# AnnaLew/pangenomix

Hardware: AMD Instinct MI355X
Metric: proteins/sec clustered at 0.8 identity + pan/core iters/sec, 400-genome set (higher is better)
Workload: dtype i32

## Files before the change

### pangenomix_amd/csrc/cluster.hip

```cpp
#include <algorithm>
#include <chrono>
#include <cstdlib>
#include <cmath>
#include <type_traits>
#include <functional>
#include <condition_variable>
#include <mutex>
#include <thread>
#include <vector>

#include "cluster_layout.h"
#include "cluster_tables.h"
#include "pgx_internal.h"

namespace {

using namespace pgxc;

constexpr uint32_t kWindowMax = 65536;
constexpr int kDiscoveryRounds = 2;
constexpr uint32_t kBlockCap = 4096;
constexpr uint32_t kBlockCapMin = 64;

constexpr uint32_t kMaxLen = 1u << 22;
// ... 1583 lines not shown
        }
        if (lane == 0) {
            uint32_t fl = F_EVAL;
            if (best_sum >= req_aas[k1r]) fl |= F_DIAG_PASS;
            if (!(br >= len2 || bl <= -len1 || bl > br)) fl |= F_BAND_OK;
            if (br - bl + 1 > kMaxBand) { fl |= F_TOO_BIG; if (fl & F_DIAG_PASS) atomicOr(err, (uint32_t)E_BAND); }
            pairs[p].best_sum = best_sum; pairs[p].band_left = bl; pairs[p].band_center = bc;
            pairs[p].band_right = br; pairs[p].flags = fl;
        }
        __syncthreads();
    }
}

enum { BK_NONE = 0, BK_DIAG = 1, BK_LEFT = 2, BK_TOP = 3 };

__device__ __forceinline__ int64_t shfl_i64(int64_t v, int src_lane) {
    const int lo = __shfl((int)(uint32_t)v, src_lane);
    const int hi = __shfl((int)(v >> 32), src_lane);
    return (int64_t)(((uint64_t)(uint32_t)hi << 32) | (uint32_t)lo);
}

__device__ int band_align_wave(const uint8_t *__restrict__ s1, const uint8_t *__restrict__ s2, int len1,
                               int len2, int bl, int bc, int br, const int8_t *__restrict__ sub ,
                               int gap_open, int gap_ext) {
    const int lane = threadIdx.x & 63;
    const int bw = br - bl + 1;
    const int j1 = lane;
    const bool col = j1 < bw;
    const int i_start = max(1, 1 - bl - j1);
    const int i_end = min(len1, len2 - bl - j1);
    const int i_start_left = max(1, 2 - bl - j1);
    const int maxd = bc - bl;
    const int dist = j1 > maxd ? j1 - maxd : maxd - j1;
    const int64_t bonus = 4 - (dist & 3);
    const int64_t gap = kScoreScale * gap_open, ext = kScoreScale * gap_ext;
    int64_t sc = 0;
    int bk = BK_NONE, id = 0;
    const int t_last = 2 * len1 + bw - 1;
    for (int t = 2; t <= t_last; ++t) {
        const int64_t l_sc_n = shfl_i64(sc, (lane + 63) & 63);
        const int l_meta = __shfl((id << 2) | bk, (lane + 63) & 63);
        const int64_t r_sc_n = shfl_i64(sc, (lane + 1) & 63);
        const int r_meta = __shfl((id << 2) | bk, (lane + 1) & 63);
        const int d = t - j1;
        const int i = d >> 1;
        if (col && !(d & 1) && i >= i_start && i <= i_end) {
            const int j = j1 + i + bl;
            const int ci = s1[i - 1], cj = s2[j - 1];
            int64_t sij = kScoreScale * (int64_t)sub[ci * kNAA1 + cj];
            if (sij > 0) sij += bonus;
            int64_t p_sc; int p_id;
            if (i - 1 >= i_start) { p_sc = sc; p_id = id; }
            else { p_sc = ext * (int64_t)((i - 1 == 0) ? (j - 1) : (i - 1)); p_id = 0; }
            int64_t best = p_sc + sij;
            int back = BK_DIAG, nid = p_id + (ci == cj);
            const int64_t gap0 = (i == len1 || j == len2) ? ext : gap;
            if (j1 > 0) {
                int64_t l_sc; int l_bk, l_id;
                if (i >= i_start_left) { l_sc = l_sc_n; l_bk = l_meta & 3; l_id = l_meta >> 2; }
                else { l_sc = ext * (int64_t)i; l_bk = BK_NONE; l_id = 0; }
                const int64_t s = l_sc + (l_bk == BK_LEFT ? ext : gap0);
                if (s > best) { best = s; back = BK_LEFT; nid = l_id; }
            }
            if (j1 + 1 < bw) {
                int64_t r_sc; int r_bk, r_id;
                if (i - 1 >= 1) { r_sc = r_sc_n; r_bk = r_meta & 3; r_id = r_meta >> 2; }
                else { r_sc = ext * (int64_t)j; r_bk = BK_NONE; r_id = 0; }
                const int64_t s = r_sc + (r_bk == BK_TOP ? ext : gap0);
                if (s > best) { best = s; back = BK_TOP; nid = r_id; }
            }
            sc = best; bk = back; id = nid;
        }
    }
    int end_lane;
    if (len2 - bl < len1) end_lane = 0;
    else if (len1 + br < len2) end_lane = bw - 1;
    else end_lane = len2 - len1 - bl;
    return __shfl(id, end_lane);
}

constexpr int kA16MaxSlot = 4096;
constexpr int kA16BigSlot = 8192;
constexpr int kScaleShift = 14;

__device__ __forceinline__ int dpp_row_shr1(int v) { return __builtin_amdgcn_update_dpp(0, v, 0x111, 0xF, 0xF, true); }
__device__ __forceinline__ int dpp_row_shl1(int v) { return __builtin_amdgcn_update_dpp(0, v, 0x101, 0xF, 0xF, true); }

__device__ __forceinline__ uint32_t lane_select(uint64_t mask, uint32_t if_set, uint32_t if_clear) {
    uint32_t d;
    asm("v_cndmask_b32_e64 %0, %1, %2, %3" : "=v"(d) : "v"(if_clear), "v"(if_set), "s"(mask));
    return d;
}
__device__ __forceinline__ uint64_t lanes_equal(uint32_t a, uint32_t b) { return __builtin_amdgcn_uicmp(a, b, 32 ); }

__device__ __forceinline__ bool pair_is_wide(int len1, int len2, int bl, int br, int max_sum) {
    return len1 + len2 > max_sum || br - bl + 1 > 32;
}

template <int kA16Slot>
__global__ __launch_bounds__(256) void align16_kernel(DevSeqs S, const uint32_t *__restrict__ rep_seq,
                                                     Pair *__restrict__ pairs, PairSel sel,
                                                     const int32_t *__restrict__ req_aa1, double cluster_thd,
                                                     uint32_t b0, unsigned long long *__restrict__ best,
                                                     uint32_t key_flag, uint32_t *__restrict__ n_wide, uint32_t second_pass) {
    __shared__ int2 tab[4][kNAA1 * kNAA1];
    __shared__ uint32_t seqbuf[16 * (kA16Slot / 4) + 32];
    __builtin_amdgcn_s_setprio(3);
    const uint32_t n = sel_count(sel);
    if (blockIdx.x * 16u >= n) return;
    if (second_pass && *n_wide == 0u) return;
    for (int c = threadIdx.x; c < 4 * kNAA1 * kNAA1; c += 256) {
        const int cc = c % (kNAA1 * kNAA1);
        const int s = S.nt ? (cc / kNAA1 == cc % kNAA1 ? 2 : -2) : (int)kBlosum62_dev[cc];
        const int v = s * (1 << kScaleShift) + (s > 0 ? c / (kNAA1 * kNAA1) + 1 : 0);
        tab[c / (kNAA1 * kNAA1)][cc] = make_int2(v * 4 + 2, cc / kNAA1 == cc % kNAA1);
    }
    __syncthreads();
    const int lane = threadIdx.x & 63, gl = lane & 15;
    const int slot = (threadIdx.x >> 6) * 4 + (lane >> 4);
    const uint8_t *sb = reinterpret_cast<const uint8_t *>(seqbuf + slot * (kA16Slot / 4));
    const int gap = (S.nt ? -6 : kGapOpen) * (1 << kScaleShift), ext = (S.nt ? -1 : kGapExt) * (1 << kScaleShift);
    constexpr int kNever = INT32_MIN / 2;

    for (uint32_t base = blockIdx.x * 16u; base < n; base += gridDim.x * 16u) {
        const uint32_t w = base + (uint32_t)slot;
        uint32_t p = 0;
        Pair pr{};
        bool fast = false;
        int len1 = 1, len2 = 1;
        uint32_t k1 = 0, k2 = 0;
        if (w < n) {
            p = sel_pair(sel, w);
            pr = pairs[p];
            k1 = pr.q; k2 = rep_seq ? rep_seq[pr.r] : pr.r;
            len1 = (int)S.len[k1]; len2 = (int)S.len[k2];
            fast = (pr.flags & (F_DIAG_PASS | F_BAND_OK | F_TOO_BIG | F_ALIGNED)) == (F_DIAG_PASS | F_BAND_OK);
            if (fast && pair_is_wide(len1, len2, pr.band_left, pr.band_right, kA16Slot - 96)) {
                fast = false;
                if (gl == 0 && !second_pass) atomicAdd(n_wide, 1u);
            }
        }
        const int bl = pr.band_left, bw = fast ? pr.band_right - pr.band_left + 1 : 0;
        int o1 = 0, o2 = 0;
        if (fast) {
            const uint32_t *p1 = S.pk + S.pk_off[k1], *p2 = S.pk + S.pk_off[k2];
            const int w1 = (len1 + 5) / 6, w2 = (len2 + 5) / 6;
            uint8_t *sbw = reinterpret_cast<uint8_t *>(seqbuf + slot * (kA16Slot / 4));
            o2 = (6 * w1 + 7) & ~7;
            for (int w = gl; w < w1; w += 16) {
                const uint32_t x = p1[w];
                for (int t = 0; t < 6; ++t) sbw[6 * w + t] = (uint8_t)((x >> (5 * t)) & 31u);
            }
            for (int w = gl; w < w2; w += 16) {
                const uint32_t x = p2[w];
                for (int t = 0; t < 6; ++t) sbw[o2 + 6 * w + t] = (uint8_t)(((x >> (5 * t)) & 31u) << 3);
            }
        }
        const int c0 = 2 * gl, c1 = c0 + 1;
        const bool v0 = c0 < bw, v1 = c1 < bw;
        const int if0 = max(0, -bl - c0), if1 = max(0, -bl - c1);
        const int ie0 = min(len1, len2 - bl - c0), ie1 = min(len1, len2 - bl - c1);
        const int bs0 = ext * (if0 > 0 ? if0 : c0 + bl), bs1 = ext * (if1 > 0 ? if1 : c1 + bl);
        const int maxd = pr.band_center - bl;
        const int d0 = c0 > maxd ? c0 - maxd : maxd - c0, d1 = c1 > maxd ? c1 - maxd : maxd - c1;
        const int2 *t0 = tab[3 - (d0 & 3)], *t1 = tab[3 - (d1 & 3)];
        const bool left0 = c0 > 0, top0 = c0 + 1 < bw, top1 = c1 + 1 < bw;
        const int trip = fast ? len1 + ((bw + 1) >> 1) : 0;

        auto res1 = [&](int i) { return (int)sb[o1 + max(i - 1, 0)]; };
        auto res2 = [&](int j) { return (int)sb[o2 + min(max(j - 1, 0), len2 - 1)]; };
        auto entry = [](const int2 *t, int c_query, int c_rep8) {
            return *reinterpret_cast<const int2 *>(__builtin_assume_aligned(
                reinterpret_cast<const char *>(t) + c_query * (kNAA1 * 8) + c_rep8, 8));
        };
        int i = -gl;
        int ci = res1(i), cje = res2(c0 + i + bl), cjo = res2(c1 + i + bl);
        int2 te = entry(t0, ci, cje), to = entry(t1, ci, cjo);
        int sc0 = 0, m0 = 0, sc1 = 0, m1 = 0;

        auto row = [&](int tau) {
            const int ci_n = res1(i + 1), cjo_n = res2(c1 + i + 1 + bl);
            const int cje_n = cjo;
            const int se = te.x >> 2, so = to.x >> 2, me = te.y, mo = to.y;
            const int l_sc = dpp_row_shr1(sc1), l_m = dpp_row_shr1(m1);
            {
                const int g0 = i == ie0 ? ext : gap;
                int bst = sc0 + se, bm = ((m0 >> 2) + me) << 2 | BK_DIAG;
                const int ls = left0 ? l_sc + ((l_m & 3) == BK_LEFT ? ext : g0) : kNever;
                if (ls > bst) { bst = ls; bm = (l_m & ~3) | BK_LEFT; }
                const int ts = top0 ? sc1 + ((m1 & 3) == BK_TOP ? ext : g0) : kNever;
                if (ts > bst) { bst = ts; bm = (m1 & ~3) | BK_TOP; }
                if (i == if0) { bst = bs0; bm = BK_NONE; }
                if (v0 && tau < trip && i >= if0 && i <= ie0) { sc0 = bst; m0 = bm; }
            }
            const int r_sc = dpp_row_shl1(sc0), r_m = dpp_row_shl1(m0);
            {
                const int g0 = i == ie1 ? ext : gap;
                int bst = sc1 + so, bm = ((m1 >> 2) + mo) << 2 | BK_DIAG;
                const int ls = sc0 + ((m0 & 3) == BK_LEFT ? ext : g0);
                if (ls > bst) { bst = ls; bm = (m0 & ~3) | BK_LEFT; }
                const int ts = top1 ? r_sc + ((r_m & 3) == BK_TOP ? ext : g0) : kNever;
                if (ts > bst) { bst = ts; bm = (r_m & ~3) | BK_TOP; }
                if (i == if1) { bst = bs1; bm = BK_NONE; }
                if (v1 && tau < trip && i >= if1 && i <= ie1) { sc1 = bst; m1 = bm; }
            }
            __builtin_amdgcn_sched_barrier(0);
            cje = cje_n; cjo = cjo_n; ci = ci_n;
            te = entry(t0, ci, cje); to = entry(t1, ci, cjo);
            ++i;
        };
        int lo = 0, hi = INT32_MAX, wtrip = trip;
        if (fast && v0) {
            lo = max(if0, v1 ? if1 : 0) + gl + 1;
            hi = min(ie0, v1 ? ie1 : ie0) + gl;
        }
        for (int d = 32; d > 0; d >>= 1) {
            lo = max(lo, __shfl_xor(lo, d)); hi = min(hi, __shfl_xor(hi, d)); wtrip = max(wtrip, __shfl_xor(wtrip, d));
        }
        wtrip = __builtin_amdgcn_readfirstlane(wtrip);
        lo = __builtin_amdgcn_readfirstlane(min(lo, wtrip)); hi = __builtin_amdgcn_readfirstlane(min(hi, wtrip));
        int tau = 0;
        for (; tau < lo; ++tau) row(tau);
        if (tau < hi) {
            constexpr uint32_t kBias = 0x80000000u;
            uint32_t G1 = (uint32_t)(gap * 4 + 1), E1 = (uint32_t)(ext * 4 + 1), G0 = (uint32_t)(gap * 4), E0 = (uint32_t)(ext * 4);
            asm volatile("" : "+v"(G1), "+v"(E1), "+v"(G0), "+v"(E0));
            const uint32_t live0 = v0 ? ~0u : 0u, live1 = v1 ? ~0u : 0u;
            auto to_key = [&](int sc, int m, uint32_t live, uint32_t &K, uint32_t &N, uint32_t &XL, uint32_t &XT) {
                const uint32_t Kc = (uint32_t)(sc * 4) + kBias;
                const int b = m & 3;
                K = Kc | (b == BK_LEFT ? 1u : (b == BK_TOP ? 0u : 2u));
                N = (uint32_t)(m >> 2);
                XL = (Kc + (b == BK_LEFT ? E1 : G1)) & live;
                XT = (Kc + (b == BK_TOP ? E0 : G0)) & live;
            };
            uint32_t K0, N0, XL0, XT0, K1, N1, XL1, XT1;
            to_key(sc0, m0, live0, K0, N0, XL0, XT0);
            to_key(sc1, m1, live1, K1, N1, XL1, XT1);
            const uint8_t *a1 = sb + o1 + i, *a2 = sb + o2 + c1 + i + bl;
            auto step = [&]() {
                const int ci_n = *a1, cjo_n = *a2;
                const int cje_n = cjo;
                ++a1; ++a2;
                {
                    const uint32_t lXL = (uint32_t)__builtin_amdgcn_update_dpp(0, (int)XL1, 0x111, 0xF, 0xF, true);
                    const uint32_t lN = (uint32_t)dpp_row_shr1((int)N1);
                    const uint32_t K = max(max((K0 & ~3u) + (uint32_t)te.x, lXL), XT1);
                    const uint32_t b = K & 3u, Kc = K & ~3u;
                    const uint64_t isL = lanes_equal(b, 1u), isT = lanes_equal(b, 0u);
                    N0 = lane_select(isL, lN, lane_select(isT, N1, N0 + (uint32_t)te.y));
                    K0 = K;
                    XL0 = (Kc + lane_select(isL, E1, G1)) & live0; XT0 = (Kc + lane_select(isT, E0, G0)) & live0;
                }
                {
                    const uint32_t rXT = (uint32_t)__builtin_amdgcn_update_dpp(0, (int)XT0, 0x101, 0xF, 0xF, true);
                    const uint32_t rN = (uint32_t)dpp_row_shl1((int)N0);
                    const uint32_t K = max(max((K1 & ~3u) + (uint32_t)to.x, XL0), rXT);
                    const uint32_t b = K & 3u, Kc = K & ~3u;
                    const uint64_t isL = lanes_equal(b, 1u), isT = lanes_equal(b, 0u);
                    N1 = lane_select(isL, N0, lane_select(isT, rN, N1 + (uint32_t)to.y));
                    K1 = K;
                    XL1 = (Kc + lane_select(isL, E1, G1)) & live1; XT1 = (Kc + lane_select(isT, E0, G0)) & live1;
                }
                __builtin_amdgcn_sched_barrier(0);
                cje = cje_n; cjo = cjo_n; ci = ci_n;
                te = entry(t0, ci, cje); to = entry(t1, ci, cjo);
                ++i;
            };
            for (; tau < hi; ++tau) step();
            asm volatile("" : "+v"(K0), "+v"(K1));
            auto from_key = [&](uint32_t K, uint32_t N, int &sc, int &m) {
                sc = (int)(K - kBias) >> 2;
                m = (int)(N << 2) | ((K & 3u) == 1u ? BK_LEFT : ((K & 3u) == 0u ? BK_TOP : BK_DIAG));
            };
            if (v0) from_key(K0, N0, sc0, m0);
            if (v1) from_key(K1, N1, sc1, m1);
        }
        for (; tau < wtrip; ++tau) row(tau);
        int ce;
        if (len2 - bl < len1) ce = 0;
        else if (len1 + pr.band_right < len2) ce = bw - 1;
        else ce = len2 - len1 - bl;
        ce = max(ce, 0);
        const int src = (lane & 48) + (ce >> 1);
        const int e0 = __shfl(m0, src), e1 = __shfl(m1, src);
        const int iden = ((ce & 1) ? e1 : e0) >> 2;
        if (fast && gl == 0) {
            const uint32_t k1r = real_of(S, k1);
            bool ok = iden >= req_aa1[k1r];
            if (ok) {
                const float pc = (float)iden / (float)len1;
                ok = !((double)pc < cluster_thd);
            }
            pairs[p].iden = iden;
            pairs[p].flags = pr.flags | F_ALIGNED | (ok ? F_ACCEPT : 0u);
            if (ok && sel.accepted_out) sel.accepted_out[k1r - b0] = 1;
            if (ok && best)
                atomicMin(&best[k1r - b0], ((unsigned long long)(k1 != k1r) << 63) | ((unsigned long long)pr.minc << 32) | key_flag | pr.r);
        }
    }
}

__global__ __launch_bounds__(256) void align_kernel(DevSeqs S, const uint32_t *__restrict__ rep_seq,
                                                   Pair *__restrict__ pairs, PairSel sel,
                                                   const int32_t *__restrict__ req_aa1, double cluster_thd,
                                                   uint32_t b0, unsigned long long *__restrict__ best,
                                                   uint32_t key_flag, int wide_only, int max_sum,
                                                   const uint32_t *__restrict__ n_wide) {
    __shared__ int8_t sub[kNAA1 * kNAA1];
    if (wide_only && *n_wide == 0u) return;
    for (int c = threadIdx.x; c < kNAA1 * kNAA1; c += 256)
        sub[c] = S.nt ? (int8_t)(c / kNAA1 == c % kNAA1 ? 2 : -2) : kBlosum62_dev[c];
    __syncthreads();
    const int gap_open = S.nt ? -6 : kGapOpen, gap_ext = S.nt ? -1 : kGapExt;
    const uint32_t n = sel_count(sel);
    const uint32_t wave = threadIdx.x >> 6, lane = threadIdx.x & 63;
    for (uint32_t w = blockIdx.x * 4 + wave; w < n; w += gridDim.x * 4) {
        const uint32_t p = sel_pair(sel, w);
        const Pair pr = pairs[p];
        if ((pr.flags & (F_DIAG_PASS | F_BAND_OK | F_TOO_BIG | F_ALIGNED)) != (F_DIAG_PASS | F_BAND_OK)) continue;
        const uint32_t k1 = pr.q, k2 = rep_seq ? rep_seq[pr.r] : pr.r;
        const int len1 = (int)S.len[k1], len2 = (int)S.len[k2];
        if (wide_only && !pair_is_wide(len1, len2, pr.band_left, pr.band_right, max_sum)) continue;
        const int iden = band_align_wave(S.res + S.off[k1], S.res + S.off[k2], len1, len2, pr.band_left,
                                         pr.band_center, pr.band_right, sub, gap_open, gap_ext);
        const uint32_t k1r = real_of(S, k1);
        bool ok = iden >= req_aa1[k1r];
        if (ok) {
            const float pc = (float)iden / (float)len1;
            ok = !((double)pc < cluster_thd);
        }
        if (lane == 0) {
            pairs[p].iden = iden;
            pairs[p].flags = pr.flags | F_ALIGNED | (ok ? F_ACCEPT : 0u);
            if (ok && sel.accepted_out) sel.accepted_out[k1r - b0] = 1;
            if (ok && best)
                atomicMin(&best[k1r - b0], ((unsigned long long)(k1 != k1r) << 63) | ((unsigned long long)pr.minc << 32) | key_flag | pr.r);
        }
    }
}

}

namespace {

constexpr unsigned kPinnedFlags = hipHostMallocCoherent | hipHostMallocMapped;
template <typename T>
struct Pinned {
    T *p = nullptr;
    size_t cap = 0;
    pgx_ctx *ctx = nullptr;
    int slot = -1;
// ... 138 lines not shown
    uint32_t w = P->alphabet == 1 ? (both ? 512u : 1024u) : 65536u;
    if (P->batch_size > 0) w = (uint32_t)P->batch_size;
    if (const char *e = std::getenv("PGX_WINDOW")) { const long v = std::atol(e); if (v > 0) w = (uint32_t)v; }
    w = std::max(w, 64u);
    w = std::min(w, kWindowMax);
    return (w + 63u) & ~63u;
}

extern "C" int pgx_cluster_greedy_dev(pgx_ctx *ctx, const uint8_t *d_residues, const uint64_t *d_offsets,
                                      uint32_t n_in, uint64_t total_in, const pgx_cluster_params *P,
                                      int32_t *out_cluster, int32_t *out_member, float *out_identity,
                                      uint8_t *out_strand, uint32_t *out_n_clusters,
                                      pgx_cluster_stats *stats, void *stream_) {
    const auto t0 = std::chrono::steady_clock::now();
    const int rc = cluster_greedy_impl(ctx, d_residues, d_offsets, n_in, total_in, P, out_cluster, out_member,
                                       out_identity, out_strand, out_n_clusters, stats, stream_);
    if (std::getenv("PGX_TRACE"))
        fprintf(stderr, "[pgx] call total (incl. clean-up)    %8.2f ms\n",
                1e3 * std::chrono::duration<double>(std::chrono::steady_clock::now() - t0).count());
    if (rc != PGX_OK && ctx) {
        (void)hipStreamSynchronize(static_cast<hipStream_t>(stream_));
        (void)hipStreamSynchronize(ctx->stream2);
        (void)hipGetLastError();
    }
    return rc;
}

static int cluster_greedy_impl(pgx_ctx *ctx, const uint8_t *d_residues, const uint64_t *d_offsets,
                               uint32_t n_in, uint64_t total_in, const pgx_cluster_params *P,
                               int32_t *out_cluster, int32_t *out_member, float *out_identity,
                               uint8_t *out_strand, uint32_t *out_n_clusters,
                               pgx_cluster_stats *stats, void *stream_) {
    PGX_REQUIRE(ctx && P, "NULL argument");
    PGX_REQUIRE(n_in == 0 || (d_residues && d_offsets), "NULL sequence arrays");
    PGX_REQUIRE(out_cluster && out_member && out_identity, "NULL output arrays");
    PGX_REQUIRE(P->alphabet == 0 || P->alphabet == 1, "alphabet must be 0 (protein) or 1 (nucleotide)");
    const bool nt = P->alphabet == 1;
    const bool both = nt && P->both_strands != 0;
    PGX_REQUIRE(P->word_len >= 2 && P->word_len <= (nt ? 11 : kMaxWordLen), "word_len must be 2..5 (protein) or 2..11 (nucleotide)");
    PGX_REQUIRE(P->identity >= 0.4 && P->identity <= 1.0, "identity must be 0.4..1.0");
    PGX_REQUIRE(P->band_width >= 1 && P->band_width <= kMaxBand, "band_width must be 1..64");
    PGX_REQUIRE(P->min_length >= P->word_len - 1, "min_length must be at least word_len - 1");
    PGX_REQUIRE(P->batch_size >= 0, "batch_size must not be negative");
    PGX_REQUIRE(P->shard_count >= 0 && (P->shard_count == 0 ? P->shard_index == 0 : (P->shard_index >= 0 && P->shard_index < P->shard_count)),
                "shard_index must be in [0, shard_count)");
    const bool native_exchange = !P->exchange && P->shard_count >= 1 && ctx->comm;
    const bool exchanging = P->exchange || native_exchange;
    PGX_REQUIRE(P->shard_count <= 1 || exchanging, "shard_count > 1 needs an exchange callback or a communicator (pgx_rccl_comm_create)");
    PGX_REQUIRE(!native_exchange || (ctx->comm_world == P->shard_count && ctx->comm_rank == P->shard_index),
                "shard_index / shard_count differ from the rank / size of the context's communicator");
    PGX_REQUIRE(!P->exchange || (P->exchange_send && P->exchange_recv),
                "the exchange callback needs exchange_send / exchange_recv (2 slots of PGX_EXCHANGE_WORDS uint64 per process, device memory)");
    PGX_HIP(hipSetDevice(ctx->device_id));
    hipStream_t st = (hipStream_t)stream_;
    const auto t_call0 = std::chrono::steady_clock::now();
    auto ms_since = [](std::chrono::steady_clock::time_point t) {
        return 1e3 * std::chrono::duration<double>(std::chrono::steady_clock::now() - t).count();
    };
    const bool trace_phases = std::getenv("PGX_TRACE") != nullptr;
    double t_mark = 0.0;
    auto phase = [&](const char *what) {
        if (!trace_phases) return;
        const double now = ms_since(t_call0);
        fprintf(stderr, "[pgx] %-28s %8.2f ms\n", what, now - t_mark);
        t_mark = now;
    };
    pgx_cluster_stats S{};
    S.n_input = n_in;
    if (out_n_clusters) *out_n_clusters = 0;
    const unsigned nth = host_threads(n_in);
    parallel_for(n_in, nth, [&](unsigned, size_t b, size_t e) {
        for (size_t i = b; i < e; ++i) {
            out_cluster[i] = -1; out_member[i] = -1; out_identity[i] = 0.f;
            if (out_strand) out_strand[i] = 0;
        }
    });
    if (n_in == 0) { if (stats) *stats = S; return PGX_OK; }

    DevBuf d_res, d_off, d_len, d_wcode, d_wmult, d_wcnt, d_aa1, d_aas, d_aan, d_lines, d_pool[2], d_idx,
        d_newbits, d_touched, d_first, d_best_own, d_rcvis, d_counters, d_visits, d_pairsW, d_pairsK, d_blk_list,
        d_ulist, d_new_list, d_flags, d_gscratch, d_order, d_list, d_gather, d_pk, d_pkoff,
        d_counters2, d_best2, d_flags2, d_pairsW2, d_gscratch2,
        d_thr, d_hugewords, d_xsend, d_xrecv,
        d_hist, d_sortcnt, d_tilesum, d_runs;
    {
        DevBuf *all[] = {&d_res, &d_off, &d_len, &d_wcode, &d_wmult, &d_wcnt, &d_aa1, &d_aas, &d_aan, &d_lines,
                         &d_pool[0], &d_pool[1], &d_idx, &d_newbits, &d_touched, &d_first, &d_best_own, &d_rcvis,
                         &d_counters, &d_visits, &d_pairsW, &d_pairsK, &d_blk_list, &d_ulist, &d_new_list, &d_flags,
                         &d_gscratch, &d_order, &d_list, &d_gather, &d_pk, &d_pkoff,
                         &d_counters2, &d_best2, &d_flags2, &d_pairsW2, &d_gscratch2, &d_thr, &d_hugewords,
                         &d_xsend, &d_xrecv, &d_hist, &d_sortcnt, &d_tilesum, &d_runs};
        int sl = 1;
        for (DevBuf *b : all) { b->ctx = ctx; b->slot = sl++; }
    }
    uint32_t n_codes = 1;
    for (int t = 0; t < P->word_len; ++t) n_codes *= nt ? 4u : (uint32_t)kNAA1;
    static_assert(kSegs == 4, "eight codes per word of the round's map");
    const uint32_t bm_words = (n_codes / 8 + 2 + 3) & ~3u;
    const bool overlap = !nt && !std::getenv("PGX_NO_OVERLAP");
    DevBuf d_in_len;
    d_in_len.ctx = ctx; d_in_len.slot = 0;
    PGX_HIP(d_in_len.alloc((size_t)n_in * 4));
    constexpr uint32_t kHistWords = H_BINS + kDevSortMaxLen + 1;
    PGX_HIP(d_hist.alloc((size_t)kHistWords * 4));
    PGX_HIP(d_idx.alloc(16));
    PGX_HIP(d_newbits.alloc(2 * (size_t)bm_words * 4 + 16));
    PGX_HIP(d_counters.alloc(C_COUNT * 4));
    PGX_HIP(d_visits.alloc(8));
    if (overlap) PGX_HIP(d_counters2.alloc(C_COUNT * 4));
    {
        ClearArgs ca{};
        auto seg = [&](DevBuf &b, size_t words) { ca.p[ca.n] = b.as<uint32_t>(); ca.words[ca.n] = (uint32_t)words; ++ca.n; };
        seg(d_hist, kHistWords);
        seg(d_newbits, 2 * (size_t)bm_words);
        seg(d_counters, C_COUNT);
        seg(d_visits, 2);
        if (overlap) seg(d_counters2, C_COUNT);
        ca.one = d_idx.as<uint32_t>();
        clear_kernel<<<1024, 256, 0, st>>>(ca);
        LAUNCH_CHECK();
    }
    {
        ProfScope prof(ctx, "seq_len_kernel", st);
        seq_len_kernel<<<(n_in + 3) / 4, 256, 0, st>>>(d_residues, d_offsets, n_in, total_in, d_in_len.as<uint32_t>());
        len_hist_kernel<<<std::min(64u, (n_in + 1023u) / 1024u), 1024, 0, st>>>(d_in_len.as<uint32_t>(), n_in, P->min_length,
                                                                               d_hist.as<uint32_t>());
    }
    LAUNCH_CHECK();
    HostVec<uint32_t> h_hist(ctx, 6, kHistWords);
    PGX_REQUIRE(h_hist.ok(), "out of host memory");
    PGX_HIP(hipMemcpyAsync(h_hist.data(), d_hist.p, (size_t)(H_BINS + kHistLds) * 4, hipMemcpyDeviceToHost, st));
    PGX_HIP(hipStreamSynchronize(st));
    const bool dev_sort = h_hist[H_OVER] == 0 && !std::getenv("PGX_HOST_PROLOGUE");
    uint32_t max_len = h_hist[H_MAX];
    if (dev_sort && max_len >= kHistLds) {
        PGX_HIP(hipMemcpyAsync(h_hist.data() + H_BINS + kHistLds, d_hist.as<uint32_t>() + H_BINS + kHistLds,
                               (size_t)(max_len + 1 - kHistLds) * 4, hipMemcpyDeviceToHost, st));
        PGX_HIP(hipStreamSynchronize(st));
    }
    phase("  seq_len + histogram + copy");
    const uint32_t *len_hist = h_hist.data() + H_BINS;
    uint32_t n = 0;
    HostVec<uint32_t> order(ctx, 1, dev_sort ? 0 : n_in);
    std::vector<uint32_t> host_hist;
    if (dev_sort) {
        for (uint32_t L = 0; L <= max_len; ++L) n += len_hist[L];
    } else {
        HostVec<uint32_t> in_len(ctx, 0, n_in);
        PGX_REQUIRE(in_len.ok() && order.ok(), "out of host memory");
        PGX_HIP(hipMemcpyAsync(in_len.data(), d_in_len.p, (size_t)n_in * 4, hipMemcpyDeviceToHost, st));
        PGX_HIP(hipStreamSynchronize(st));
        max_len = 0;
        {
            std::vector<uint32_t> mx(nth, 0u);
            parallel_for(n_in, nth, [&](unsigned t, size_t b, size_t e) {
                uint32_t m = 0;
                for (size_t i = b; i < e; ++i) m = std::max(m, in_len[i]);
                mx[t] = m;
            });
            for (uint32_t m : mx) max_len = std::max(max_len, m);
        }
        if (max_len > kMaxLen) {
            pgx_set_error("pgx_cluster_greedy: sequence of %u residues exceeds the supported maximum %u", max_len, kMaxLen);
            return PGX_ERR_CAPACITY;
        }
        const size_t n_bkt = (size_t)max_len + 2;
        std::vector<uint32_t> bucket(n_bkt * nth, 0);
        parallel_for(n_in, nth, [&](unsigned t, size_t b, size_t e) {
            uint32_t *h = bucket.data() + n_bkt * t;
            for (size_t i = b; i < e; ++i)
                if ((int)in_len[i] > P->min_length) h[max_len - in_len[i]]++;
        });
        host_hist.assign((size_t)max_len + 1, 0u);
        for (size_t l = 0; l <= max_len; ++l)
// ... 107 lines not shown
    PGX_HIP(d_aas.alloc((size_t)n * 4));
    PGX_HIP(d_aan.alloc((size_t)n * 4));
    PGX_HIP(d_lines.alloc((size_t)n_codes * sizeof(IndexLine)));
    PGX_HIP(hipMemsetAsync(d_lines.p, 0, (size_t)n_codes * sizeof(IndexLine), st));
    PGX_HIP(d_best_own.alloc((size_t)window_cap * 8));
    PGX_HIP(d_rcvis.alloc((size_t)window_cap * 8));
    PGX_HIP(d_blk_list.alloc((size_t)kBlockCap * 4));
    PGX_HIP(d_ulist.alloc((size_t)window_cap * 4));
    PGX_HIP(d_new_list.alloc((size_t)window_cap * 4));
    PGX_HIP(d_flags.alloc(4 * (size_t)window_cap));
    PGX_HIP(d_list.alloc((size_t)pair_cap_k * 4));
    PGX_HIP(d_gather.alloc((size_t)pair_cap_k * sizeof(Pair)));
    PGX_HIP(d_pairsW.alloc((size_t)pair_cap * sizeof(Pair)));
    PGX_HIP(d_pairsK.alloc((size_t)pair_cap_k * sizeof(Pair)));
    if (need_gscratch) PGX_HIP(d_gscratch.alloc((size_t)diag_grid * gs_stride * 4));
    if (overlap) {
        if (!exchanging) PGX_HIP(d_best2.alloc((size_t)window_cap * 8));
        PGX_HIP(d_flags2.alloc(4 * (size_t)window_cap));
        PGX_HIP(d_pairsW2.alloc((size_t)pair_cap * sizeof(Pair)));
        if (need_gscratch) PGX_HIP(d_gscratch2.alloc((size_t)diag_grid * gs_stride * 4));
    }
    int pool_cur = 0;
    uint64_t pool_cap = 0;
    auto ensure_pool = [&](uint64_t entries, hipStream_t on) -> int {
        const uint64_t need = 8 * entries + 4096;
        if (need <= pool_cap) return PGX_OK;
        if (need > 0xFFFFFFF0ull) { pgx_set_error("pgx_cluster_greedy: word index too large for 32-bit pool offsets"); return PGX_ERR_CAPACITY; }
        const uint64_t want = std::min<uint64_t>(0xFFFFFFF0ull, need + need / 2);
        DevBuf &nb_ = d_pool[pool_cur ^ 1];
        PGX_HIP(nb_.alloc(want * 4));
        if (pool_cap) PGX_HIP(hipMemcpyAsync(nb_.p, d_pool[pool_cur].p, pool_cap * 4, hipMemcpyDeviceToDevice, on));
        pool_cur ^= 1;
        pool_cap = want;
        return PGX_OK;
    };
    PGX_HIP(d_order.alloc((size_t)n * 4));
    if (dev_sort) {
        uint32_t per = kSortShare;
        while ((uint64_t)((n_in + per - 1) / per) * n_runs > kSortCells) per *= 2;
        const uint32_t n_shares = (n_in + per - 1) / per, cells = n_shares * n_runs, tiles = (cells + kScanTile - 1) / kScanTile;
        PGX_HIP(d_sortcnt.alloc((size_t)cells * 4));
        PGX_HIP(d_tilesum.alloc((size_t)tiles * 4));
        uint32_t *const cnt = d_sortcnt.as<uint32_t>(), *const in_len = d_in_len.as<uint32_t>();
        ProfScope prof(ctx, "length_sort_kernels", st);
        ClearArgs ca{};
        ca.p[0] = cnt; ca.words[0] = cells; ca.n = 1;
        clear_kernel<<<std::min(2048u, (cells + 255u) / 256u), 256, 0, st>>>(ca);
        sort_count_kernel<<<(n_in + 255) / 256, 256, 0, st>>>(in_len, n_in, P->min_length, max_len, per, n_shares, cnt);
        tile_sum_kernel<<<tiles, 256, 0, st>>>(cnt, cells, d_tilesum.as<uint32_t>());
        tile_scan_kernel<<<tiles, 256, 0, st>>>(cnt, cells, d_tilesum.as<uint32_t>());
        sort_place_kernel<<<(n_shares + 3) / 4, 256, 0, st>>>(in_len, n_in, P->min_length, max_len, per, n_shares, cnt, n,
                                                              d_order.as<uint32_t>());
        LAUNCH_CHECK();
        PGX_HIP(hipMemcpyAsync(order.data(), d_order.p, (size_t)n * 4, hipMemcpyDeviceToHost, st));
    } else {
        PGX_HIP(hipMemcpyAsync(d_order.p, order.data(), (size_t)n * 4, hipMemcpyHostToDevice, st));
    }
    {
        const size_t runs_bytes = 2 * ((size_t)n_runs + 1) * 8;
        PGX_HIP(d_runs.alloc(runs_bytes));
        PGX_HIP(hipMemcpyAsync(d_runs.p, h_runs.data(), runs_bytes, hipMemcpyHostToDevice, st));
        const uint64_t *const dr_off = d_runs.as<uint64_t>();
        const uint32_t *const dr_pos = reinterpret_cast<const uint32_t *>(dr_off + n_runs + 1), *const dr_pk = dr_pos + n_runs + 1;
        layout_kernel<<<nv / 256 + 1, 256, 0, st>>>(dr_off, dr_pos, dr_pk, n_runs, max_len, n, nv, d_len.as<uint32_t>(),
                                                    d_off.as<uint64_t>(), d_pkoff.as<uint32_t>());
        LAUNCH_CHECK();
    }
    {
        ProfScope prof(ctx, "encode_gather_kernel", st);
        encode_gather_kernel<<<(n + 3) / 4, 256, 0, st>>>(d_residues, d_offsets, d_order.as<uint32_t>(),
                                                          d_off.as<uint64_t>(), d_res.as<uint8_t>(), n, nt ? 1 : 0);
        if (both)
            revcomp_kernel<<<(n + 3) / 4, 256, 0, st>>>(d_res.as<uint8_t>(), d_off.as<uint64_t>(),
                                                        d_len.as<uint32_t>(), n);
        pack5_kernel<<<(nv + 3) / 4, 256, 0, st>>>(d_res.as<uint8_t>(), d_off.as<uint64_t>(), d_len.as<uint32_t>(),
                                                   d_pkoff.as<uint32_t>(), nv, d_pk.as<uint32_t>());
    }
    LAUNCH_CHECK();
    {
        PGX_HIP(d_thr.alloc(3 * ((size_t)max_len + 1) * 4));
        PGX_HIP(hipMemcpyAsync(d_thr.p, h_thr.data(), 3 * ((size_t)max_len + 1) * 4, hipMemcpyHostToDevice, st));
        thresholds_kernel<<<(n + 255) / 256, 256, 0, st>>>(d_len.as<uint32_t>(), n, d_thr.as<int32_t>(), max_len + 1,
                                                          d_aa1.as<int32_t>(), d_aas.as<int32_t>(), d_aan.as<int32_t>());
        LAUNCH_CHECK();
    }
    phase("alloc + sort + layout + encode (enq)");
    {
        const int wl = P->word_len;
        auto first_with_words_le = [&](uint32_t cap) { return pgxc::first_with_words_le(run_pos, max_len, cap, wl); };
        const uint32_t k32 = first_with_words_le(32768), k8 = first_with_words_le(8192),
                       k2 = first_with_words_le(2048), k1k = first_with_words_le(1023), k5 = first_with_words_le(512);
        int rc;
        uint8_t *r8 = d_res.as<uint8_t>(); uint64_t *o64 = d_off.as<uint64_t>(); uint32_t *l32 = d_len.as<uint32_t>();
        uint32_t *wc = d_wcode.as<uint32_t>(); uint16_t *wm = d_wmult.as<uint16_t>(); uint32_t *wn = d_wcnt.as<uint32_t>();
        const int base = nt ? 4 : kNAA1;
        for (uint32_t half = 0; half < (both ? 2u : 1u); ++half) {
            const uint32_t o = half * n;
            if (k32) {
                uint32_t slots = 65536;
                while (slots < 2u * max_len) slots *= 2;
                const uint32_t per_launch = std::min(k32, std::max(1u, (uint32_t)((256ull << 20) / ((uint64_t)slots * 8))));
                PGX_HIP(d_hugewords.alloc((size_t)per_launch * slots * 8));
                ProfScope prof(ctx, "words_kernel", st);
                for (uint32_t a = 0; a < k32; a += per_launch)
                    words_huge_kernel<<<std::min(per_launch, k32 - a), 1024, 0, st>>>(r8, o64, l32, o + a, o + std::min(k32, a + per_launch), wl, base,
                                                                                       nt, d_hugewords.as<uint32_t>(), slots, wc, wm, wn,
                                                                                       d_counters.as<uint32_t>() + C_ERR);
                LAUNCH_CHECK();
            }
            if ((rc = launch_words<32768, 1024>(ctx, st, r8, o64, l32, o + k32, o + k8, wl, base, nt, wc, wm, wn))) return rc;
            if ((rc = launch_words<8192, 1024>(ctx, st, r8, o64, l32, o + k8, o + k2, wl, base, nt, wc, wm, wn))) return rc;
            if ((rc = launch_words_hash<2048, 256>(ctx, st, r8, o64, l32, o + k2, o + k1k, wl, base, nt, wc, wm, wn))) return rc;
            if (k5 > k1k) {
                ProfScope prof(ctx, "words_kernel", st);
                words_wave_kernel<2048><<<(k5 - k1k + 3) / 4, 256, 0, st>>>(r8, o64, l32, o + k1k, o + k5, wl, base, nt, wc, wm, wn);
                LAUNCH_CHECK();
            }
            if (n > k5) {
                ProfScope prof(ctx, "words_kernel", st);
                words_wave_kernel<1024><<<(n - k5 + 3) / 4, 256, 0, st>>>(r8, o64, l32, o + k5, o + n, wl, base, nt, wc, wm, wn);
                LAUNCH_CHECK();
            }
        }
    }
    DevSeqs DS{d_res.as<uint8_t>(), d_off.as<uint64_t>(), d_len.as<uint32_t>(),
               d_wcode.as<uint32_t>(), d_wmult.as<uint16_t>(), d_wcnt.as<uint32_t>(),
               d_pk.as<uint32_t>(), d_pkoff.as<uint32_t>(), n, nt ? 4 : kNAA1, nt ? 4 : 2, nt ? 1 : 0, mshift};
    HostVec<uint32_t> h_wcnt(ctx, 8, n);
    PGX_REQUIRE(h_wcnt.ok(), "out of host memory");
    PGX_HIP(hipMemcpyAsync(h_wcnt.data(), d_wcnt.p, (size_t)n * 4, hipMemcpyDeviceToHost, st));

    phase("word lists (enqueue)");
    fill_host_layout();
    phase("host lengths + offsets");
    uint64_t max_window_words = 0;
    uint32_t max_chunks = 1;
    {
        Chunks C;
        size_t nf = 0;
        for (uint32_t b0 = 0, nbw; b0 < n; b0 += nbw) {
            while (nf < flush_at.size() && flush_at[nf] <= b0) ++nf;
            nbw = form_window(b0, C, nf < flush_at.size() ? flush_at[nf] : n);
            max_window_words = std::max<uint64_t>(max_window_words, h_off[b0 + nbw] - h_off[b0]);
            max_chunks = std::max(max_chunks, C.n);
        }
        if (!flush_at.empty())
            max_window_words = std::max<uint64_t>(max_window_words, h_off[std::min(n, window_cap)]);
    }
    if (chunking && flush_at.empty())
        max_window_words = std::max<uint64_t>(max_window_words,
            std::min<uint64_t>(h_off[std::min(n, window_cap)], (uint64_t)kMaxChunks * std::max<uint64_t>(chunk_words, max_len)));
    PGX_REQUIRE(max_window_words < 0xFFFFFFF0ull, "window too large");
    PGX_HIP(d_touched.alloc((max_window_words + 16) * sizeof(Deferred)));
    if (chunking && n > window_cap / 2) max_chunks = kMaxChunks;
    uint32_t tag_stride = 1;
    while (tag_stride < max_chunks) tag_stride *= 2;
    PGX_HIP(d_first.alloc((size_t)tag_stride * n_codes * 4 + 16));
    std::vector<uint32_t> rep_seq;
    HostVec<int32_t> cluster_of(ctx, 9, n, -1);
    HostVec<int32_t> iden_of(ctx, 10, n, -1);
    PGX_REQUIRE(cluster_of.ok() && iden_of.ok(), "out of host memory");
    Pinned<Pair> hW, hK;
    Pinned<unsigned long long> h_best, h_rcvis;
    Pinned<uint32_t> h_cnt, h_blk, h_new, h_list, h_push;
    Pinned<Pair> h_gather;
    hW.bind(ctx, 0); hK.bind(ctx, 1); h_best.bind(ctx, 2); h_cnt.bind(ctx, 3); h_blk.bind(ctx, 4);
// ... 93 lines not shown
    for (uint32_t cursor = 0, nb = 0; cursor < n;) {
        if (!sweeping && next_flush < flush_at.size() && cursor == flush_at[next_flush]) {
            ++next_flush;
            sweeping = true; sweep_at = cursor;
            int rc = drain(); if (rc) return rc;
        }
        const bool sweep = sweeping;
        const uint32_t b0 = sweep ? sweep_at : cursor;
        nb = form_window(b0, chunks, sweep || next_flush >= flush_at.size() ? n : flush_at[next_flush]);
        const int set = overlap ? (int)(S.sweeps & 1u) : 0;
        const hipStream_t st = set ? ctx->stream2 : st_main;
        uint32_t *const dc = dc_set[set];
        unsigned long long *const d_best = d_best_set[set];
        uint8_t *const d_done = d_flags_set[set], *const d_inblk = d_done + window_cap;
        uint8_t *const d_hascand = d_done + 2 * (size_t)window_cap, *const d_accepted = d_done + 3 * (size_t)window_cap;
        Pinned<Pair> &hW_w = set ? hW2 : hW;
        Pinned<unsigned long long> &h_best_w = set ? h_best2 : h_best;
        Pinned<uint32_t> &h_ccnt_w = set ? h_ccnt2 : h_ccnt;
        uint32_t *const d_gs = (set ? d_gscratch2 : d_gscratch).as<uint32_t>();
        if (overlap && S.sweeps > 0)
            PGX_HIP(hipStreamWaitEvent(st, ev.strike[set ^ 1], 0));
        bool strike_recorded = false;
        const uint32_t ns = both ? 2 * nb : nb;
        const uint32_t n_reps = (uint32_t)rep_seq.size();
        const uint64_t window_words = h_off[b0 + nb] - h_off[b0];
        { int rc = ensure_pool(S.rep_words + pending_words + window_words, st); if (rc) return rc; }
        uint32_t *d_poolp = d_pool[pool_cur].as<uint32_t>();
        if (nt) {
            const uint64_t need = (uint64_t)ns * ((uint64_t)n_reps + nb) + 1024;
            if (need > (400ull << 20)) {
                pgx_set_error("pgx_cluster_greedy: %llu candidate pairs in one window exceed the supported maximum",
                              (unsigned long long)need);
                return PGX_ERR_CAPACITY;
            }
            if (need > pair_cap) {
                PGX_HIP(spin_sync(st));
                if (deferred) { int rc = deferred(); deferred = nullptr; if (rc) return rc; }
                pair_cap = (uint32_t)(need + need / 2);
                PGX_HIP(d_pairsW.alloc((size_t)pair_cap * sizeof(Pair)));
            }
        }
        S.sweeps++;
        const auto t_sweep0 = std::chrono::steady_clock::now();
        const uint64_t blocks_before = n_blocks;
        const int two_len = 2 * (int)h_len[b0];
        const int a16_slot = two_len <= 1024 - 96 ? 1024 : (two_len <= 1536 - 96 ? 1536 : (two_len <= 2048 - 96 ? 2048 : (two_len <= 3072 - 96 ? 3072 : kA16MaxSlot)));
        Pair *pairsW = (set ? d_pairsW2 : d_pairsW).as<Pair>();
        FilterArgs FA{};
        FA.lines = d_lines.as<IndexLine>(); FA.pool = d_poolp; FA.newbits = d_newbits.as<uint32_t>();
        FA.d_round_lo = dc + C_SEG0; FA.d_round_hi = dc + C_NEW; FA.epoch = 0;
        FA.b0 = b0; FA.nbq = nb; FA.ns = ns; FA.shard_index = shard_index; FA.shard_count = shard_count;
        FA.req_aan = d_aan.as<int32_t>(); FA.best = d_best; FA.done = d_done;
        FA.pairs = pairsW; FA.n_pairs = dc + C_NW; FA.pair_cap = pair_cap;
        FA.visits = d_visits.as<unsigned long long>(); FA.rc_visits = d_rcvis_p; FA.err = dc + C_ERR;
        FA.qlist = nullptr; FA.d_nq = nullptr; FA.mark = nullptr; FA.count_visits = 1u;
        FA.lean = stats == nullptr && !std::getenv("PGX_NO_LEAN") ? 1u : 0u;

        window_init_kernel<<<(window_cap + 255) / 256, 256, 0, st>>>(dc, d_best, both ? d_rcvis_p : nullptr, d_done, window_cap);
        if (!flush_at.empty() && next_flush > 0)
            mark_absent_kernel<<<(nb + 255) / 256, 256, 0, st>>>(h_taken.p + b0, nb, d_done, d_best);
        LAUNCH_CHECK();
        auto begin_host_side = [&]() -> int {
            if (deferred) { int rc = deferred(); deferred = nullptr; if (rc) return rc; }
            for (uint32_t q = 0; q < nb; ++q) status[q] = cluster_of[b0 + q] >= 0 ? ST_ABSENT : ST_OPEN;
            return PGX_OK;
        };
        bool older_reps = false;
        auto evaluate = [&](Pair *pairs, const PairSel &sel, unsigned long long *best_arr, uint32_t grid_hint) -> int {
            const uint32_t dg = grid_hint ? std::min(diag_grid, grid_hint) : diag_grid;
            const uint32_t ag = grid_hint ? std::min(align_grid, (grid_hint + 15) / 16) : align_grid;
            {
                ProfScope prof(ctx, "diag_kernel", st);
                auto kern = h_len[b0] > packed_len ? diag_kernel<64, unsigned long long>
                            : (h_len[b0] <= kDiagLdsSmall ? diag_kernel<kDiagLdsSmall, uint32_t>
                               : (h_len[b0] <= 2 * kDiagLdsSmall ? diag_kernel<2 * kDiagLdsSmall, uint32_t> : diag_kernel<kDiagLdsCap, uint32_t>));
                kern<<<dg, 64, 0, st>>>(DS, nullptr, pairs, sel, d_aa1.as<int32_t>(), d_aas.as<int32_t>(),
                                        P->band_width, P->identity, d_gs, gs_stride, gs_cells, dc + C_WIDE, dc + C_ERR);
            }
            LAUNCH_CHECK();
            {
                ProfScope prof(ctx, "align_kernel", st);
                auto kern = a16_slot == 1024 ? align16_kernel<1024> : (a16_slot == 1536 ? align16_kernel<1536> : (a16_slot == 2048 ? align16_kernel<2048>
                            : (a16_slot == 3072 ? align16_kernel<3072> : align16_kernel<kA16MaxSlot>)));
                kern<<<ag, 256, 0, st>>>(DS, nullptr, pairs, sel, d_aa1.as<int32_t>(), P->identity, b0, best_arr, 0u, dc + C_WIDE, 0u);
                const bool big_pass = a16_slot == kA16MaxSlot && two_len > kA16MaxSlot - 96;
                const bool may_be_wide = older_reps || two_len > a16_slot - 96 || P->band_width > 32;
                if (big_pass)
                    align16_kernel<kA16BigSlot><<<ag, 256, 0, st>>>(DS, nullptr, pairs, sel, d_aa1.as<int32_t>(), P->identity, b0, best_arr,
                                                                    0u, dc + C_WIDE, 1u);
                if (may_be_wide)
                    align_kernel<<<grid_hint ? std::min(align_grid, (grid_hint + 3) / 4) : align_grid, 256, 0, st>>>(
                        DS, nullptr, pairs, sel, d_aa1.as<int32_t>(), P->identity, b0, best_arr, 0u, 1, (big_pass ? kA16BigSlot : a16_slot) - 96, dc + C_WIDE);
            }
            LAUNCH_CHECK();
            return PGX_OK;
        };
        auto exchange_best = [&]() -> int {
            if (!exchanging) return PGX_OK;
            ++n_exchanges;
            exchange_prepare_kernel<<<1, 1, 0, st>>>(dc, pair_cap, d_best,
                                                     inject_rank == (int)shard_index && inject_at == n_exchanges ? (uint32_t)E_PAIRS : 0u);
            if (native_exchange) {
                const int rc = pgx_rccl_all_gather_u64(ctx, x_send + (size_t)set * PGX_EXCHANGE_WORDS,
                                                       const_cast<unsigned long long *>(x_recv) + (size_t)set * shard_count * PGX_EXCHANGE_WORDS,
                                                       PGX_EXCHANGE_WORDS, st);
                if (rc) return rc;
            } else if (P->exchange(P->exchange_user, (void *)st, set) != 0) {
                pgx_set_error("pgx_cluster_greedy: the exchange callback failed in the window at %u", b0);
                return PGX_ERR_INTERNAL;
            }
            min_rows_kernel<<<(nb + 255) / 256, 256, 0, st>>>(
                x_recv + (size_t)set * shard_count * PGX_EXCHANGE_WORDS,
                shard_count, PGX_EXCHANGE_WORDS, nb, d_best, dc + C_ERR);
            LAUNCH_CHECK();
            return PGX_OK;
        };
        auto evaluate_round = [&]() -> int {
            const PairSel sel{dc + C_EVAL0, dc + C_NW, pair_cap, nullptr, 0, nullptr, nullptr, nullptr, b0, 0, 0};
            int rc = evaluate(pairsW, sel, d_best, 0);
            if (rc) return rc;
            return exchange_best();
        };
        if (b0 > 0) {
            {
                ProfScope prof(ctx, "filter_kernel<all>", st);
                auto kern = nt ? filter_kernel<true, false> : filter_kernel<false, false>;
                kern<<<std::min(filter_grid, (ns + 3) / 4), 256, 0, st>>>(DS, FA);
            }
            LAUNCH_CHECK();
            filter_walk_words += window_words * (both ? 2 : 1) / shard_count;
            older_reps = true;
            int rc = evaluate_round();
            older_reps = false;
            if (rc) return rc;
        }
        auto index_append = [&](const uint32_t *list, const uint32_t *d_lo, const uint32_t *d_hi) -> int {
            ++epoch_idx;
            uint32_t *const map = d_newbits.as<uint32_t>() + (size_t)(epoch_idx & 1u) * bm_words;
            uint32_t *const next_map = d_newbits.as<uint32_t>() + (size_t)((epoch_idx + 1u) & 1u) * bm_words;
            ProfScope prof(ctx, "index_append", st);
            index_append_kernel<<<512, 256, 0, st>>>(DS, list, d_lo, d_hi, d_lines.as<IndexLine>(), epoch_idx,
                                                     map, b0, nb, d_touched.as<Deferred>(),
                                                     dc + C_TOUCH, (uint32_t)max_window_words, dc + C_ERR);
            index_grow_kernel<<<256, 256, 0, st>>>(d_lines.as<IndexLine>(), d_poolp, d_idx.as<uint32_t>(),
                                                   (uint32_t)pool_cap, d_touched.as<Deferred>(), dc + C_TOUCH,
                                                   (uint32_t)max_window_words, dc + C_ERR);
            index_place_kernel<<<256, 256, 0, st>>>(d_lines.as<IndexLine>(), d_poolp, d_touched.as<Deferred>(),
                                                    dc + C_TOUCH, (uint32_t)max_window_words, reinterpret_cast<uint4 *>(next_map),
                                                    bm_words / 4);
            LAUNCH_CHECK();
            return PGX_OK;
        };
        auto filter_new_and_evaluate = [&](const uint32_t *d_lo, const uint32_t *d_hi) -> int {
            FilterArgs F = FA;
            F.epoch = epoch_idx; F.d_round_lo = d_lo; F.d_round_hi = d_hi;
            F.newbits = d_newbits.as<uint32_t>() + (size_t)(epoch_idx & 1u) * bm_words;
            {
                ProfScope prof(ctx, "filter_kernel<new>", st);
                auto kern = nt ? filter_kernel<true, true> : filter_kernel<false, true>;
                kern<<<std::min(filter_grid, (ns + 3) / 4), 256, 0, st>>>(DS, F);
            }
            LAUNCH_CHECK();
            filter_walk_words += window_words * (both ? 2 : 1) / shard_count;
            return evaluate_round();
        };
        uint32_t n_listed = 0;
        if (sweep) { int rc = begin_host_side(); if (rc) return rc; }
        if (!sweep) {
        if (overlap && S.sweeps > 1)
            PGX_HIP(hipStreamWaitEvent(st, ev.post[set ^ 1], 0));
        static const int n_disc = std::getenv("PGX_ROUNDS") ? std::atoi(std::getenv("PGX_ROUNDS")) : kDiscoveryRounds;
// ... 391 lines not shown
```

Before: 16.54 million.

## Precompute align16 score table, skew LDS slots, prefetch residues two rows ahead

The scaled substitution table is now built once into a device buffer by a separate kernel, and each align16 block copies it into LDS with 16-byte loads instead of recomputing it. Sequence slots for odd-numbered groups are offset by 64 bytes, presumably to spread LDS bank use across neighbouring slots. The inner anti-diagonal step now loads residues two rows ahead and looks up the next table entries before the DP update, with the loop unrolled by two, so LDS latency can hide behind the arithmetic. This adds LDS footprint and register pressure, and it relies on the 96-byte slack per slot to keep the look-ahead reads inside the slot.

```diff
diff --git a/pangenomix_amd/csrc/cluster.hip b/pangenomix_amd/csrc/cluster.hip
--- a/pangenomix_amd/csrc/cluster.hip
+++ b/pangenomix_amd/csrc/cluster.hip
@@ -1689,6 +1689,7 @@
 constexpr int kA16MaxSlot = 4096;
 constexpr int kA16BigSlot = 8192;
 constexpr int kScaleShift = 14;
+constexpr int kA16Skew = 64;
 
 __device__ __forceinline__ int dpp_row_shr1(int v) { return __builtin_amdgcn_update_dpp(0, v, 0x111, 0xF, 0xF, true); }
 __device__ __forceinline__ int dpp_row_shl1(int v) { return __builtin_amdgcn_update_dpp(0, v, 0x101, 0xF, 0xF, true); }
@@ -1704,28 +1705,35 @@
     return len1 + len2 > max_sum || br - bl + 1 > 32;
 }
 
+constexpr int kA16TabEntries = 4 * kNAA1 * kNAA1;
+static_assert(kA16TabEntries * sizeof(int2) % 16 == 0, "copied in 16-byte pieces");
+__global__ __launch_bounds__(256) void align16_table_kernel(int nt, int2 *__restrict__ out) {
+    const int c = blockIdx.x * 256 + threadIdx.x;
+    if (c >= kA16TabEntries) return;
+    const int cc = c % (kNAA1 * kNAA1);
+    const int s = nt ? (cc / kNAA1 == cc % kNAA1 ? 2 : -2) : (int)kBlosum62_dev[cc];
+    const int v = s * (1 << kScaleShift) + (s > 0 ? c / (kNAA1 * kNAA1) + 1 : 0);
+    out[c] = make_int2(v * 4 + 2, cc / kNAA1 == cc % kNAA1);
+}
+
 template <int kA16Slot>
-__global__ __launch_bounds__(256) void align16_kernel(DevSeqs S, const uint32_t *__restrict__ rep_seq,
+__global__ __launch_bounds__(256) void align16_kernel(DevSeqs S, const int4 *__restrict__ tab_src, const uint32_t *__restrict__ rep_seq,
                                                      Pair *__restrict__ pairs, PairSel sel,
                                                      const int32_t *__restrict__ req_aa1, double cluster_thd,
                                                      uint32_t b0, unsigned long long *__restrict__ best,
                                                      uint32_t key_flag, uint32_t *__restrict__ n_wide, uint32_t second_pass) {
-    __shared__ int2 tab[4][kNAA1 * kNAA1];
-    __shared__ uint32_t seqbuf[16 * (kA16Slot / 4) + 32];
+    __shared__ __attribute__((aligned(16))) int2 tab[4][kNAA1 * kNAA1];
+    __shared__ uint32_t seqbuf[16 * (kA16Slot / 4) + kA16Skew / 4 + 32];
+    static_assert(sizeof(tab) + sizeof(seqbuf) <= 160 * 1024, "one workgroup's LDS");
     __builtin_amdgcn_s_setprio(3);
     const uint32_t n = sel_count(sel);
     if (blockIdx.x * 16u >= n) return;
     if (second_pass && *n_wide == 0u) return;
-    for (int c = threadIdx.x; c < 4 * kNAA1 * kNAA1; c += 256) {
-        const int cc = c % (kNAA1 * kNAA1);
-        const int s = S.nt ? (cc / kNAA1 == cc % kNAA1 ? 2 : -2) : (int)kBlosum62_dev[cc];
-        const int v = s * (1 << kScaleShift) + (s > 0 ? c / (kNAA1 * kNAA1) + 1 : 0);
-        tab[c / (kNAA1 * kNAA1)][cc] = make_int2(v * 4 + 2, cc / kNAA1 == cc % kNAA1);
-    }
+    for (int c = threadIdx.x; c < (int)(sizeof(tab) / 16); c += 256) reinterpret_cast<int4 *>(&tab[0][0])[c] = tab_src[c];
     __syncthreads();
     const int lane = threadIdx.x & 63, gl = lane & 15;
     const int slot = (threadIdx.x >> 6) * 4 + (lane >> 4);
-    const uint8_t *sb = reinterpret_cast<const uint8_t *>(seqbuf + slot * (kA16Slot / 4));
+    const uint8_t *sb = reinterpret_cast<const uint8_t *>(seqbuf + slot * (kA16Slot / 4) + (slot & 1) * (kA16Skew / 4));
     const int gap = (S.nt ? -6 : kGapOpen) * (1 << kScaleShift), ext = (S.nt ? -1 : kGapExt) * (1 << kScaleShift);
     constexpr int kNever = INT32_MIN / 2;
 
@@ -1752,7 +1760,7 @@
         if (fast) {
             const uint32_t *p1 = S.pk + S.pk_off[k1], *p2 = S.pk + S.pk_off[k2];
             const int w1 = (len1 + 5) / 6, w2 = (len2 + 5) / 6;
-            uint8_t *sbw = reinterpret_cast<uint8_t *>(seqbuf + slot * (kA16Slot / 4));
+            uint8_t *sbw = const_cast<uint8_t *>(sb);
             o2 = (6 * w1 + 7) & ~7;
             for (int w = gl; w < w1; w += 16) {
                 const uint32_t x = p1[w];
@@ -1778,7 +1786,7 @@
         auto res2 = [&](int j) { return (int)sb[o2 + min(max(j - 1, 0), len2 - 1)]; };
         auto entry = [](const int2 *t, int c_query, int c_rep8) {
             return *reinterpret_cast<const int2 *>(__builtin_assume_aligned(
-                reinterpret_cast<const char *>(t) + c_query * (kNAA1 * 8) + c_rep8, 8));
+                reinterpret_cast<const char *>(t) + __umul24(c_query, kNAA1 * 8) + c_rep8, 8));
         };
         int i = -gl;
         int ci = res1(i), cje = res2(c0 + i + bl), cjo = res2(c1 + i + bl);
@@ -1845,10 +1853,14 @@
             to_key(sc0, m0, live0, K0, N0, XL0, XT0);
             to_key(sc1, m1, live1, K1, N1, XL1, XT1);
             const uint8_t *a1 = sb + o1 + i, *a2 = sb + o2 + c1 + i + bl;
+            static_assert(96 - (12 + 17) >= kA16Skew, "reads two rows ahead stay inside a skewed slot");
+            int ci1 = a1[0], cjo1 = a2[0];
+            asm volatile("" : "+v"(ci1), "+v"(cjo1));
             auto step = [&]() {
-                const int ci_n = *a1, cjo_n = *a2;
-                const int cje_n = cjo;
+                const int ci2 = a1[1], cjo2 = a2[1];
+                const int2 te_n = entry(t0, ci1, cjo), to_n = entry(t1, ci1, cjo1);
                 ++a1; ++a2;
+                __builtin_amdgcn_sched_barrier(0);
                 {
                     const uint32_t lXL = (uint32_t)__builtin_amdgcn_update_dpp(0, (int)XL1, 0x111, 0xF, 0xF, true);
                     const uint32_t lN = (uint32_t)dpp_row_shr1((int)N1);
@@ -1870,11 +1882,11 @@
                     XL1 = (Kc + lane_select(isL, E1, G1)) & live1; XT1 = (Kc + lane_select(isT, E0, G0)) & live1;
                 }
                 __builtin_amdgcn_sched_barrier(0);
-                cje = cje_n; cjo = cjo_n; ci = ci_n;
-                te = entry(t0, ci, cje); to = entry(t1, ci, cjo);
+                te = te_n; to = to_n; cjo = cjo1; ci1 = ci2; cjo1 = cjo2;
                 ++i;
             };
-            for (; tau < hi; ++tau) step();
+            for (; tau + 2 <= hi; tau += 2) { step(); step(); }
+            if (tau < hi) { step(); ++tau; }
             asm volatile("" : "+v"(K0), "+v"(K1));
             auto from_key = [&](uint32_t K, uint32_t N, int &sc, int &m) {
                 sc = (int)(K - kBias) >> 2;
@@ -2179,14 +2191,15 @@
         d_ulist, d_new_list, d_flags, d_gscratch, d_order, d_list, d_gather, d_pk, d_pkoff,
         d_counters2, d_best2, d_flags2, d_pairsW2, d_gscratch2,
         d_thr, d_hugewords, d_xsend, d_xrecv,
-        d_hist, d_sortcnt, d_tilesum, d_runs;
+        d_hist, d_sortcnt, d_tilesum, d_runs,
+        d_a16tab;
     {
         DevBuf *all[] = {&d_res, &d_off, &d_len, &d_wcode, &d_wmult, &d_wcnt, &d_aa1, &d_aas, &d_aan, &d_lines,
                          &d_pool[0], &d_pool[1], &d_idx, &d_newbits, &d_touched, &d_first, &d_best_own, &d_rcvis,
                          &d_counters, &d_visits, &d_pairsW, &d_pairsK, &d_blk_list, &d_ulist, &d_new_list, &d_flags,
                          &d_gscratch, &d_order, &d_list, &d_gather, &d_pk, &d_pkoff,
                          &d_counters2, &d_best2, &d_flags2, &d_pairsW2, &d_gscratch2, &d_thr, &d_hugewords,
-                         &d_xsend, &d_xrecv, &d_hist, &d_sortcnt, &d_tilesum, &d_runs};
+                         &d_xsend, &d_xrecv, &d_hist, &d_sortcnt, &d_tilesum, &d_runs, &d_a16tab};
         int sl = 1;
         for (DevBuf *b : all) { b->ctx = ctx; b->slot = sl++; }
     }
@@ -2460,6 +2473,9 @@
         PGX_HIP(hipMemcpyAsync(d_thr.p, h_thr.data(), 3 * ((size_t)max_len + 1) * 4, hipMemcpyHostToDevice, st));
         thresholds_kernel<<<(n + 255) / 256, 256, 0, st>>>(d_len.as<uint32_t>(), n, d_thr.as<int32_t>(), max_len + 1,
                                                           d_aa1.as<int32_t>(), d_aas.as<int32_t>(), d_aan.as<int32_t>());
+        LAUNCH_CHECK();
+        PGX_HIP(d_a16tab.alloc(kA16TabEntries * sizeof(int2)));
+        align16_table_kernel<<<(kA16TabEntries + 255) / 256, 256, 0, st>>>(nt ? 1 : 0, d_a16tab.as<int2>());
         LAUNCH_CHECK();
     }
     phase("alloc + sort + layout + encode (enq)");
@@ -2719,11 +2735,11 @@
                 ProfScope prof(ctx, "align_kernel", st);
                 auto kern = a16_slot == 1024 ? align16_kernel<1024> : (a16_slot == 1536 ? align16_kernel<1536> : (a16_slot == 2048 ? align16_kernel<2048>
                             : (a16_slot == 3072 ? align16_kernel<3072> : align16_kernel<kA16MaxSlot>)));
-                kern<<<ag, 256, 0, st>>>(DS, nullptr, pairs, sel, d_aa1.as<int32_t>(), P->identity, b0, best_arr, 0u, dc + C_WIDE, 0u);
+                kern<<<ag, 256, 0, st>>>(DS, d_a16tab.as<int4>(), nullptr, pairs, sel, d_aa1.as<int32_t>(), P->identity, b0, best_arr, 0u, dc + C_WIDE, 0u);
                 const bool big_pass = a16_slot == kA16MaxSlot && two_len > kA16MaxSlot - 96;
                 const bool may_be_wide = older_reps || two_len > a16_slot - 96 || P->band_width > 32;
                 if (big_pass)
-                    align16_kernel<kA16BigSlot><<<ag, 256, 0, st>>>(DS, nullptr, pairs, sel, d_aa1.as<int32_t>(), P->identity, b0, best_arr,
+                    align16_kernel<kA16BigSlot><<<ag, 256, 0, st>>>(DS, d_a16tab.as<int4>(), nullptr, pairs, sel, d_aa1.as<int32_t>(), P->identity, b0, best_arr,
                                                                     0u, dc + C_WIDE, 1u);
                 if (may_be_wide)
                     align_kernel<<<grid_hint ? std::min(align_grid, (grid_hint + 3) / 4) : align_grid, 256, 0, st>>>(
```

Result: no change. 16.69 million, median of 4 (+0.9%).
